# hila-chefer/Transformer-Explainability

Hardware: NVIDIA H100
Metric: explanations_per_sec (higher is better)
Workload: dtype f32

## Files before the change

include/te_b200.h:

```cpp
#ifndef TE_B200_H
#define TE_B200_H

#ifdef __cplusplus
extern "C" {
#endif

#if defined(__GNUC__)
#define TE_API __attribute__((visibility("default")))
#else
#define TE_API
#endif

#define TE_OK 0
#define TE_ERR_ARG (-1)
#define TE_ERR_WORKSPACE (-2)
#define TE_ERR_CUDA (-3)
#define TE_ERR_UNSUPPORTED (-4)

#define TE_FLAG_ZPLUS_TENSOR_CORES 1u
#define TE_FLAG_ROLLOUT_FUSED 2u
#define TE_FLAG_KEEP_ALL_CAMS 4u
#define TE_FLAG_LINEAR_TENSOR_CORES 16u
#define TE_FLAG_ATTN_TENSOR_CORES 32u
#define TE_FLAG_ZPLUS_BF16 64u
// ... 74 lines not shown
#define TE_BERT_ARCH_ROBERTA 1
#define TE_BERT_ARCH_DISTILBERT 2

TE_API int te_bert_num_weights(const te_bert_config* cfg);
TE_API const char* te_bert_weight_name(const te_bert_config* cfg, int i);
TE_API long long te_bert_weight_numel(const te_bert_config* cfg, int i);
TE_API long long te_bert_weight_offset(const te_bert_config* cfg, int i);
TE_API long long te_bert_weight_total(const te_bert_config* cfg);
TE_API long long te_bert_derived_total(const te_bert_config* cfg);
TE_API int te_bert_prepare_derived(const te_bert_config* cfg, const float* weights, float* derived, void* stream);
TE_API long long te_bert_workspace_bytes(const te_bert_config* cfg, int batch, int seq);

TE_API int te_bert_forward(const te_bert_config* cfg, const float* weights, const float* derived,
                    const long long* input_ids, const long long* attention_mask, const long long* token_type_ids,
                    int batch, int seq, unsigned flags, float* logits, void* workspace, long long workspace_bytes,
                    void* stream);
TE_API int te_bert_attribute(const te_bert_config* cfg, const float* weights, const float* derived, int batch, int seq,
                             int* index, int start_layer, float alpha, unsigned flags, float* maps, void* workspace,
                             long long workspace_bytes, void* stream);
TE_API int te_bert_explain(const te_bert_config* cfg, const float* weights, const float* derived,
                    const long long* input_ids, const long long* attention_mask, const long long* token_type_ids,
                    int batch, int seq, int* index, int start_layer, unsigned flags, float* maps, float* logits,
                    void* workspace, long long workspace_bytes, void* stream);
TE_API int te_bert_tensor(const te_bert_config* cfg, int batch, int seq, void* workspace, const char* name, int layer,
                   float** ptr, long long dims[4], long long strides[4]);

TE_API int te_linear_relprop(const float* x, const float* w, const float* bias, const float* y, const float* r, float* out,
                             float* scratch, int rows, int in_features, int out_features, float alpha, unsigned flags,
                             void* stream);
TE_API int te_add_relprop(const float* x1, const float* x2, const float* r, float* r1, float* r2, void* scratch,
                   int batch, long long per_sample, void* stream);
TE_API int te_clone_relprop(const float* x, const float* r1, const float* r2, const float* r3, float* out, long long n,
                     void* stream);
TE_API int te_matmul_av_relprop(const float* p, const float* v, const float* r, float* rp, float* rv, float* scratch,
                         int bh, int n, int d, void* stream);
TE_API int te_matmul_qk_relprop(const float* q, const float* k, const float* r, float* rq, float* rk, float* scratch,
                         int bh, int n, int d, void* stream);
TE_API int te_index_select_relprop(const float* x, const float* r, float* out, int batch, int n, int d, void* stream);
TE_API long long te_patch_embed_relprop_workspace_bytes(int batch, int in_chans, int img_size, int patch_size, int dim);
TE_API int te_patch_embed_relprop(const float* images, const float* weight, const float* r, int batch, int in_chans,
                           int img_size, int patch_size, int dim, float* r_pixels, float* r_sum, void* workspace,
                           long long workspace_bytes, void* stream);

TE_API int te_relevance_heatmap(const float* maps, int batch, int grid, int scale, float* out, void* stream);
TE_API int te_render_overlay(const float* images, const float* heat, int batch, int h, int w, int otsu, unsigned char* out,
                             int* thresholds, void* stream);
TE_API int te_head_reduce(const float* a, const float* g, const float* head_w, int batch, int heads, int n, int ld, int mode,
                   float* out, void* stream);
TE_API int te_head_region_mean(const float* g, int batch, int heads, int n, int ld, int r0, int r1, int c0, int c1, float* out,
                        void* stream);

TE_API long long te_rollout_workspace_bytes(int layers, int batch, int n);
TE_API int te_attribution_rollout(const float* grad, const float* cam, int layers, int batch, int heads, int n, int ld,
                           int start_layer, int normalize, unsigned flags, float* joint, float* row0,
                           void* workspace, long long workspace_bytes, void* stream);
TE_API int te_compute_rollout_attention(const float* mats, int layers, int batch, int n, int start_layer, int normalize,
                                 float* joint, void* workspace, long long workspace_bytes, void* stream);

TE_API int te_f16_block_split(const float* x, int rows, int cols, void* hi, void* lo, float* scale_inv, void* stream);

TE_API int te_linear_forward(const float* x, const float* w, const float* bias, const float* e0, float* y, float* y2,
                             float* scratch, int rows, int in_features, int out_features, int epi, unsigned flags,
                             void* stream);
TE_API int te_linear_backward(const float* dy, const float* w, const float* e0, float* dx, float* scratch, int rows,
                              int in_features, int out_features, int epi, unsigned flags, void* stream);
TE_API int te_layernorm_split(const float* x, const float* w, const float* b, float* y, float* mean, float* rstd, void* hi,
// ... 71 lines not shown
```

transformer_explainability_b200/_lib.py:

```python
import ctypes
import os

HERE = os.path.dirname(os.path.abspath(__file__))
LIB_PATH = os.path.join(HERE, "lib", "libte_b200.so")

c_int, c_ll, c_uint, c_void_p, c_char_p, c_float = (ctypes.c_int, ctypes.c_longlong, ctypes.c_uint, ctypes.c_void_p,
                                                    ctypes.c_char_p, ctypes.c_float)


class TeVitConfig(ctypes.Structure):
    _fields_ = [("img_size", c_int), ("patch_size", c_int), ("in_chans", c_int), ("num_classes", c_int),
                ("dim", c_int), ("depth", c_int), ("heads", c_int), ("mlp_dim", c_int), ("distilled", c_int),
                ("eps_block", c_float), ("eps_final", c_float)]


class TeBertConfig(ctypes.Structure):
    _fields_ = [("vocab_size", c_int), ("max_position", c_int), ("type_vocab", c_int), ("hidden", c_int),
                ("layers", c_int), ("heads", c_int), ("intermediate", c_int), ("num_labels", c_int),
                ("layer_norm_eps", c_float), ("arch", c_int), ("pad_token_id", c_int)]


BERT_ARCH_BERT = 0
BERT_ARCH_ROBERTA = 1
BERT_ARCH_DISTILBERT = 2
# ... 28 lines not shown
    "te_version": (c_int, []),
    "te_kernel_launch_count": (c_ll, []),
    "te_vit_num_weights": (c_int, [_CFG]),
    "te_vit_weight_name": (c_char_p, [_CFG, c_int]),
    "te_vit_weight_numel": (c_ll, [_CFG, c_int]),
    "te_vit_weight_offset": (c_ll, [_CFG, c_int]),
    "te_vit_weight_total": (c_ll, [_CFG]),
    "te_vit_workspace_bytes": (c_ll, [_CFG, c_int]),
    "te_vit_forward": (c_int, [_CFG, _P, _P, _P, c_int, c_uint, _P, _P, c_ll, _P]),
    "te_vit_derived_total": (c_ll, [_CFG]),
    "te_vit_prepare_derived": (c_int, [_CFG, _P, _P, _P]),
    "te_vit_attribute": (c_int, [_CFG, _P, _P, c_int, _P, c_int, c_float, c_uint, _P, _P, c_ll, _P]),
    "te_vit_explain": (c_int, [_CFG, _P, _P, _P, c_int, _P, c_int, c_uint, _P, _P, _P, c_ll, _P]),
    "te_vit_tensor": (c_int, [_CFG, c_int, _P, c_char_p, c_int, ctypes.POINTER(_P), ctypes.POINTER(c_ll),
                              ctypes.POINTER(c_ll)]),
    "te_set_option": (c_int, [c_char_p, c_int]),
    "te_vit_relprop_pixels": (c_int, [_CFG, _P, _P, c_int, c_uint, _P, _P, _P, c_ll, _P]),
    "te_bert_num_weights": (c_int, [_BCFG]),
    "te_bert_weight_name": (c_char_p, [_BCFG, c_int]),
    "te_bert_weight_numel": (c_ll, [_BCFG, c_int]),
    "te_bert_weight_offset": (c_ll, [_BCFG, c_int]),
    "te_bert_weight_total": (c_ll, [_BCFG]),
    "te_bert_derived_total": (c_ll, [_BCFG]),
    "te_bert_prepare_derived": (c_int, [_BCFG, _P, _P, _P]),
    "te_bert_workspace_bytes": (c_ll, [_BCFG, c_int, c_int]),
    "te_bert_forward": (c_int, [_BCFG, _P, _P, _P, _P, _P, c_int, c_int, c_uint, _P, _P, c_ll, _P]),
    "te_bert_attribute": (c_int, [_BCFG, _P, _P, c_int, c_int, _P, c_int, c_float, c_uint, _P, _P, c_ll, _P]),
    "te_bert_explain": (c_int, [_BCFG, _P, _P, _P, _P, _P, c_int, c_int, _P, c_int, c_uint, _P, _P, _P, c_ll, _P]),
    "te_bert_tensor": (c_int, [_BCFG, c_int, c_int, _P, c_char_p, c_int, ctypes.POINTER(_P), ctypes.POINTER(c_ll),
                               ctypes.POINTER(c_ll)]),
    "te_linear_relprop": (c_int, [_P, _P, _P, _P, _P, _P, _P, c_int, c_int, c_int, c_float, c_uint, _P]),
    "te_add_relprop": (c_int, [_P, _P, _P, _P, _P, _P, c_int, c_ll, _P]),
    "te_clone_relprop": (c_int, [_P, _P, _P, _P, _P, c_ll, _P]),
    "te_matmul_av_relprop": (c_int, [_P, _P, _P, _P, _P, _P, c_int, c_int, c_int, _P]),
    "te_matmul_qk_relprop": (c_int, [_P, _P, _P, _P, _P, _P, c_int, c_int, c_int, _P]),
    "te_index_select_relprop": (c_int, [_P, _P, _P, c_int, c_int, c_int, _P]),
    "te_patch_embed_relprop_workspace_bytes": (c_ll, [c_int, c_int, c_int, c_int, c_int]),
    "te_patch_embed_relprop": (c_int, [_P, _P, _P, c_int, c_int, c_int, c_int, c_int, _P, _P, _P, c_ll, _P]),
    "te_relevance_heatmap": (c_int, [_P, c_int, c_int, c_int, _P, _P]),
    "te_render_overlay": (c_int, [_P, _P, c_int, c_int, c_int, c_int, _P, _P, _P]),
    "te_head_reduce": (c_int, [_P, _P, _P, c_int, c_int, c_int, c_int, c_int, _P, _P]),
    "te_head_region_mean": (c_int, [_P, c_int, c_int, c_int, c_int, c_int, c_int, c_int, c_int, _P, _P]),
    "te_rollout_workspace_bytes": (c_ll, [c_int, c_int, c_int]),
    "te_attribution_rollout": (c_int, [_P, _P, c_int, c_int, c_int, c_int, c_int, c_int, c_int, c_uint, _P, _P, _P,
                                       c_ll, _P]),
    "te_compute_rollout_attention": (c_int, [_P, c_int, c_int, c_int, c_int, c_int, _P, _P, c_ll, _P]),
    "te_f16_block_split": (c_int, [_P, c_int, c_int, _P, _P, _P, _P]),
    "te_linear_forward": (c_int, [_P, _P, _P, _P, _P, _P, _P, c_int, c_int, c_int, c_int, c_uint, _P]),
    "te_linear_backward": (c_int, [_P, _P, _P, _P, _P, c_int, c_int, c_int, c_int, c_uint, _P]),
    "te_layernorm_split": (c_int, [_P, _P, _P, _P, _P, _P, _P, _P, _P, c_int, c_int, c_float, _P]),
    "te_tc_zplus_s": (c_int, [_P, _P, _P, _P, _P, _P, _P, _P, _P, c_int, c_int, c_int, c_uint, _P]),
    "te_tc_attention_nn": (c_int, [_P, c_ll, _P, c_ll, c_int, c_int, c_int, c_int, _P, c_int, _P, c_float, c_int, c_int, _P]),
    "te_tc_attention_nk": (c_int, [_P, c_int, c_int, _P, c_ll, c_int, c_int, c_int, _P, c_int, _P, c_float, c_int, c_int, _P]),
    "te_perturb_workspace_bytes": (c_ll, [c_int, c_ll]),
    "te_perturb_images": (c_int, [_P, _P, c_int, c_int, c_ll, ctypes.POINTER(c_int), c_int, c_int, ctypes.POINTER(c_float),
                                  ctypes.POINTER(c_float), _P, _P, c_ll, _P]),
    "te_logit_stats": (c_int, [_P, _P, c_int, c_int, _P, _P, _P, _P, _P]),
    "te_sort_workspace_bytes": (c_ll, [c_ll, c_int]),
    "te_sort_keys_u32": (c_int, [_P, _P, c_ll, c_int, _P, c_ll, _P]),
    "te_seg_workspace_bytes": (c_ll, [c_int, c_int, c_int]),
    "te_seg_metrics": (c_int, [_P, _P, c_int, c_int, c_int, c_float, _P, _P, _P, _P, _P, _P, _P, _P, c_ll, _P]),
    "te_pr_curve_workspace_bytes": (c_ll, [c_ll]),
    "te_pr_curve": (c_int, [_P, c_ll, _P, _P, _P, _P, _P, c_ll, _P]),
    "te_eraser_workspace_bytes": (c_ll, [c_int, c_ll, c_ll]),
    "te_eraser_rationales": (c_int, [_P, c_int, c_int, _P, _P, _P, _P, _P, c_int, _P, c_int, _P, _P, _P, _P, c_ll, _P]),
    "te_eraser_reduce_workspace_bytes": (c_ll, [c_int, c_ll, c_int]),
# ... 66 lines not shown
```

transformer_explainability_b200/csrc/te_api.cu:

```cuda
#include <stdlib.h>
#include <string.h>
#include <atomic>
#include <string>

#include "../../include/te_b200.h"
#include "te_engine_util.h"
#include "te_kernels.h"
#include "te_rollout.h"
#include "te_zplus.h"
#include "te_gemm_tc.h"

static thread_local std::string g_last_error;
void te_set_last_error(const char* msg) { g_last_error = msg ? msg : ""; }

static std::atomic<long long> g_launches{0};
void te_count_launch() { g_launches.fetch_add(1, std::memory_order_relaxed); }
extern "C" long long te_kernel_launch_count(void) { return g_launches.load(); }

extern "C" const char* te_last_error(void) { return g_last_error.c_str(); }
extern "C" int te_version(void) { return 101; }

#define ST(s) reinterpret_cast<cudaStream_t>(s)
#define REQ(c, msg) do { if (!(c)) { te_set_last_error(msg); return TE_ERR_ARG; } } while (0)

// ... 132 lines not shown

extern "C" int te_linear_relprop(const float* x, const float* w, const float* bias, const float* y, const float* r, float* out,
                                 float* scratch, int rows, int in_features, int out_features, float alpha, unsigned flags,
                                 void* stream) {
    REQ(x && w && r && out && scratch && rows > 0 && in_features > 0 && out_features > 0, "te_linear_relprop: bad argument");
    REQ(isfinite(alpha), "te_linear_relprop: alpha must be finite");
    const bool lrp = (flags & TE_FLAG_RULES_LRP) != 0;
    const float* derived = nullptr;
    float* xabs = nullptr;
    if ((flags & (lrp ? TE_FLAG_RULES_LRP_TC : TE_FLAG_ZPLUS_TENSOR_CORES)) &&
        te_tc_zplus_supported(rows, in_features, out_features, in_features)) {
        const TcScratch c = tc_scratch(scratch, (long long)rows * out_features, in_features, out_features, 0);
        TE_TRY(te_tc_prepare_weights(w, c.derived, in_features, out_features, ST(stream)));
        derived = c.derived;
        if (y) xabs = c.op;
    }
    return te_linear_rule_relprop(lrp, x, in_features, w, derived, r, out_features, out, scratch, rows, in_features, out_features,
                                  ST(stream), y, out_features, bias, y ? te_zplus_from_flags(flags) : ZplusVariant{}, 0, xabs,
                                  alpha);
}

extern "C" int te_add_relprop(const float* x1, const float* x2, const float* r, float* r1, float* r2, void* scratch,
                              int batch, long long per_sample, void* stream) {
    REQ(x1 && x2 && r && r1 && r2 && batch > 0 && per_sample > 0, "te_add_relprop: bad argument");
    return te_launch_add_relprop(x1, x2, r, r1, r2, reinterpret_cast<double*>(scratch), batch, per_sample, ST(stream));
}

extern "C" int te_clone_relprop(const float* x, const float* r1, const float* r2, const float* r3, float* out,
                                long long n, void* stream) {
    REQ(x && r1 && r2 && out && n > 0, "te_clone_relprop: bad argument");
    return te_launch_clone_relprop(x, r1, r2, r3, out, n, ST(stream));
}

extern "C" int te_index_select_relprop(const float* x, const float* r, float* out, int batch, int n, int d,
                                       void* stream) {
    REQ(x && r && out && batch > 0 && n > 0 && d > 0, "te_index_select_relprop: bad argument");
    return te_launch_index_select_relprop(x, r, nullptr, out, batch, n, d, ST(stream));
}

extern "C" int te_matmul_av_relprop(const float* p_, const float* v, const float* r, float* rp, float* rv,
                                    float* scratch, int bh, int n, int d, void* stream) {
    REQ(p_ && v && r && rp && rv && scratch && bh > 0 && n > 0 && d > 0 && d % 4 == 0, "te_matmul_av_relprop: bad argument");
    cudaStream_t st = ST(stream);
    const long long nn = (long long)n * n, nd = (long long)n * d;
    TeGemm g = g0(bh);
    g.A = p_; g.lda = n; g.sA1 = nn; g.B = v; g.ldb = d; g.sB1 = nd; g.C = scratch; g.ldc = d; g.sC1 = nd;
    g.M = n; g.N = d; g.K = n;
    TE_TRY(te_gemm_launch(g, TE_L_K, TE_L_MN, TE_XF_NONE, TE_EPI_STORE, st));
    TE_TRY(te_launch_sd(r, scratch, scratch, (long long)bh * nd, st));
    g = g0(bh);
    g.A = scratch; g.lda = d; g.sA1 = nd; g.B = v; g.ldb = d; g.sB1 = nd; g.C = rp; g.ldc = n; g.sC1 = nn;
    g.E0 = p_; g.lde0 = n; g.sE1 = nn; g.M = n; g.N = n; g.K = d;
    TE_TRY(te_gemm_launch(g, TE_L_K, TE_L_K, TE_XF_NONE, TE_EPI_MUL, st));
    g = g0(bh);
    g.A = p_; g.lda = n; g.sA1 = nn; g.B = scratch; g.ldb = d; g.sB1 = nd; g.C = rv; g.ldc = d; g.sC1 = nd;
    g.E0 = v; g.lde0 = d; g.sE1 = nd; g.M = n; g.N = d; g.K = n;
    TE_TRY(te_gemm_launch(g, TE_L_MN, TE_L_MN, TE_XF_NONE, TE_EPI_MUL, st));
    return TE_OK;
}

extern "C" int te_matmul_qk_relprop(const float* q, const float* k, const float* r, float* rq, float* rk,
                                    float* scratch, int bh, int n, int d, void* stream) {
    REQ(q && k && r && rq && rk && scratch && bh > 0 && n > 0 && d > 0, "te_matmul_qk_relprop: bad argument");
    cudaStream_t st = ST(stream);
    const long long nn = (long long)n * n, nd = (long long)n * d;
    TeGemm g = g0(bh);
// ... 124 lines not shown
```

transformer_explainability_b200/csrc/te_bert.cu:

```cuda
#include <string.h>

#include <algorithm>

#include "../../include/te_b200.h"
#include "te_engine_util.h"
#include "te_gemm_tc.h"
#include "te_kernels.h"
#include "te_rollout.h"
#include "te_zplus.h"

using namespace te_util;

namespace {

constexpr int kMaxDepth = 64;

struct Dims {
    int B, N, NP, D, H, dh, F, C, L, V, P, T, arch, pad;
    long long M;
    float eps;
};

static bool make_dims(const te_bert_config* c, int B, int S, Dims& d) {
    if (!c || c->layers <= 0 || c->layers > kMaxDepth || c->heads <= 0 || c->hidden % c->heads != 0 || c->hidden % 8 != 0 ||
// ... 326 lines not shown
        TE_TRY(linear_bwd_tc(tw.qkv, dqkv, lw.qkvw, dxn, nullptr, d.M, d.D, 3 * d.D, TE_EPI_STORE, st, sel.btf, &sel.bfs));
        TE_TRY(te_launch_add2(dxn, dsx, dxa, MD, st));
    }

    if (flags & TE_FLAG_GRADIENTS_ONLY) return TE_OK;
    const long long layer_stride = d.L > 1 ? (long long)(ws.layer[1].G - ws.layer[0].G) : 0;
    if (grad_rollout) {
        TE_TRY(te_rollout_layers(ws.layer[0].G, ws.layer[0].P, layer_stride, d.L, d.B, d.H, d.N, d.NP, d.NP, start_layer,
                                 0, flags, ws.mats, ws.joint[0], ws.joint[1], nullptr, maps, 0,
                                 0, st));
        if (cudaMemset2DAsync(maps, sizeof(float) * d.N, 0, sizeof(float), d.B, st) != cudaSuccess) {
            te_set_last_error("te_bert_attribute: clearing element 0 of the maps failed");
            return TE_ERR_CUDA;
        }
        return TE_OK;
    }

    float* R = ws.tD[0]; float* R1 = ws.tD[1]; float* R2 = ws.tD[2]; float* R3 = ws.tD[3];
    float* RF = ws.tF[0]; float* SF = ws.tF[1]; float* S = ws.t3D[0]; float* Rqkv = ws.t3D[1];
    double* addp = sel.lrp ? nullptr : ws.addpart;
    TE_TRY(te_linear_rule_relprop(sel.lrp, ws.pooled, d.D, w.clsw, nullptr, ws.seed, d.C, ws.rpool, ws.shead, d.B, d.D, d.C, st,
                                  nullptr, 0, nullptr, sel.zv, 0, nullptr, alpha));
    TE_TRY(te_linear_rule_relprop(sel.lrp, ws.h_last, (long long)d.N * d.D, w.poolw, nullptr, ws.rpool, d.D, ws.rfirst, ws.shead,
                                  d.B, d.D, d.D, st, nullptr, 0, nullptr, sel.zv, 0, nullptr, alpha));
    TE_TRY(te_launch_index_select_relprop(ws.h_last, ws.rfirst, nullptr, R, d.B, d.N, d.D, st));

    for (int l = d.L - 1; l >= sel.low; --l) {
        LayerAct& a = ws.layer[l];
        const LayerW& lw = w.layer[l];
        const DerivedW dw = bind_derived(d, sel.dbase, l);
        const bool top = (l == d.L - 1) && te_engine_cls_rows();
        const long long zr = top ? d.B : d.M;
        const long long sD = top ? (long long)d.N * d.D : d.D, sF = top ? (long long)d.N * d.F : d.F;
        TE_TRY(te_launch_add_relprop(a.d2, a.ao, R, R1, R2, addp, d.B, (long long)d.N * d.D, st));
        TE_TRY(te_linear_rule_relprop(sel.lrp, a.g, sF, lw.w2, dw.w2, R1, sD, RF, S, zr, d.F, d.D, st, a.d2, sD, lw.b2, sel.zv, sF,
                                      SF, alpha));
        TE_TRY(te_linear_rule_relprop(sel.lrp, a.ao, sD, lw.w1, dw.w1, RF, sF, R1, SF, zr, d.D, d.F, st, a.hpre, sF, lw.b1, sel.zv,
                                      sD, S, alpha));
        TE_TRY(te_launch_clone_relprop(a.ao, R1, R2, nullptr, R, MD, st));
        TE_TRY(te_launch_add_relprop(a.d1, a.h, R, R1, R2, addp, d.B, (long long)d.N * d.D, st));
        if (top) TE_TRY(te_launch_fill(R3, 0.f, MD, st));
        TE_TRY(te_linear_rule_relprop(sel.lrp, a.ctx, sD, lw.ow, dw.o, R1, sD, R3, S, zr, d.D, d.D, st, a.d1, sD, lw.ob, sel.zv, sD,
                                      S + MD, alpha));
        const bool last = (l == sel.low && !(flags & TE_FLAG_RELPROP_TO_INPUT));
        TE_TRY(attn_relprop_pv(sel, d.B, d.H, d.N, d.NP, d.dh, a.qkv, a.P, R3, a.ctx, S, a.cam, Rqkv, last, st));
        if (last) break;
        TE_TRY(attn_nn(sel.atc, d.B, d.H, d.N, d.NP, d.dh, a.qkv, 3 * d.D, a.qkv + d.D, 3 * d.D, ws.tA[0], nullptr, scale,
                       TE_EPI_STORE, st));
        TE_TRY(te_launch_add_relprop_keymask(ws.tA[0], ws.maskadd, a.cam, ws.tA[1], addp, d.B, d.H, d.N, d.NP, st));
        TE_TRY(attn_relprop_qk(sel, d.B, d.H, d.N, d.NP, d.dh, a.qkv, ws.tA[1], ws.tA[0], Rqkv, st));
        TE_TRY(te_linear_rule_relprop(sel.lrp, a.h, d.D, lw.qkvw, dw.q, Rqkv, 3 * d.D, R, S, d.M, d.D, d.D, st, a.qkv, 3 * d.D,
                                      lw.qkvb, sel.zv, 0, S + MD, alpha));
        TE_TRY(te_linear_rule_relprop(sel.lrp, a.h, d.D, lw.qkvw + DD, dw.k, Rqkv + d.D, 3 * d.D, R1, S, d.M, d.D, d.D, st,
                                      a.qkv + d.D, 3 * d.D, lw.qkvb + d.D, sel.zv, 0, S + MD, alpha));
        TE_TRY(te_linear_rule_relprop(sel.lrp, a.h, d.D, lw.qkvw + 2 * DD, dw.v, Rqkv + 2 * d.D, 3 * d.D, R3, S, d.M, d.D, d.D, st,
                                      a.qkv + 2 * d.D, 3 * d.D, lw.qkvb + 2 * d.D, sel.zv, 0, S + MD, alpha));
        TE_TRY(te_launch_clone_relprop(a.h, R, R1, R3, SF, MD, st));
        TE_TRY(te_launch_clone_relprop(a.h, SF, R2, nullptr, R, MD, st));
    }

    TE_TRY(te_rollout_layers(ws.layer[0].G, ws.layer[0].cam, layer_stride, d.L, d.B, d.H, d.N, d.NP, d.NP, start_layer,
                             1, flags, ws.mats, ws.joint[0], ws.joint[1], nullptr, maps, 0,
                             1, st));
    return TE_OK;
}

extern "C" int te_bert_explain(const te_bert_config* cfg, const float* weights, const float* derived,
                               const long long* input_ids, const long long* attention_mask,
                               const long long* token_type_ids, int batch, int seq, int* index, int start_layer,
                               unsigned flags, float* maps, float* logits, void* workspace, long long workspace_bytes,
                               void* stream) {
    TE_TRY(te_bert_forward(cfg, weights, derived, input_ids, attention_mask, token_type_ids, batch, seq, flags, logits,
                           workspace, workspace_bytes, stream));
    return te_bert_attribute(cfg, weights, derived, batch, seq, index, start_layer, 1.f, flags, maps, workspace, workspace_bytes,
                             stream);
}

extern "C" int te_bert_tensor(const te_bert_config* cfg, int batch, int seq, void* workspace, const char* name, int layer,
                              float** ptr, long long dims[4], long long strides[4]) {
    Dims d; Workspace ws;
    if (!workspace || !name || !ptr) return TE_ERR_ARG;
    if (batch <= 0 || !make_dims(cfg, batch, seq, d)) return TE_ERR_ARG;
    carve(d, reinterpret_cast<char*>(workspace), ws);
    const std::string n(name);
    const View set{ptr, dims, strides};
    if (n == "logits") return set(ws.logits, d.B, d.C, 1, 1, d.C, 1, 1, 1);
    if (n == "relevance_in") return set(ws.tD[0], d.B, d.N, d.D, 1, (long long)d.N * d.D, d.D, 1, 1);
    if (n.rfind("tmp_d", 0) == 0 && n.size() == 6 && n[5] >= '0' && n[5] <= '3')
        return set(ws.tD[n[5] - '0'], d.B, d.N, d.D, 1, (long long)d.N * d.D, d.D, 1, 1);
    if (n.rfind("tmp_f", 0) == 0 && n.size() == 6 && n[5] >= '0' && n[5] <= '1')
        return set(ws.tF[n[5] - '0'], d.B, d.N, d.F, 1, (long long)d.N * d.F, d.F, 1, 1);
// ... 24 lines not shown
```

transformer_explainability_b200/csrc/te_kernels.h:

```cpp
#pragma once
#include "te_common.cuh"
#include "te_gemm.cuh"

int te_launch_im2col(const float* img, float* patches, int B, int C, int H, int W, int P, cudaStream_t st);
int te_launch_assemble_tokens(const float* patch_out, const float* cls, const float* dist, const float* pos,
                              float* x, int B, int N, int D, int n_prefix, cudaStream_t st);
int te_launch_layernorm(const float* x, const float* w, const float* b, float* y, float* mean, float* rstd,
                        long long rows, int D, float eps, cudaStream_t st);
int te_launch_layernorm_split(const float* x, const float* w, const float* b, float* y, float* mean, float* rstd,
                              long long rows, int D, float eps, float* split, float* scale, cudaStream_t st);
int te_launch_layernorm_bwd(const float* dy, const float* x, const float* w, const float* mean, const float* rstd,
                            const float* dres, float* dx, long long rows, int D, cudaStream_t st);
int te_launch_layernorm_bwd_strided(const float* dy, long long dy_stride, const float* x, long long x_stride,
                                    const float* w, float eps, float* dx, long long dx_stride, int rows, int D,
                                    cudaStream_t st);
int te_launch_softmax(float* s, long long rows, int N, int ld, cudaStream_t st);
int te_launch_softmax_bwd(const float* p, const float* dp, float* ds, long long rows, int N, int ld, float scale,
                          cudaStream_t st);
int te_launch_argmax(const float* logits, int* index, int B, int C, int only_negative, cudaStream_t st);
int te_launch_average2(const float* a, const float* b, float* out, long long n, cudaStream_t st);
int te_launch_onehot(const int* index, float* seed, int B, int C, float value, cudaStream_t st);
int te_launch_sd(const float* a, const float* b, float* out, long long n, cudaStream_t st);
int te_launch_clone_relprop(const float* x, const float* r1, const float* r2, const float* r3, float* out,
                            long long n, cudaStream_t st);
#define TE_ADD_SPLIT 16
int te_launch_add_relprop(const float* x1, const float* x2, const float* r, float* r1, float* r2, double* partial,
                          int B, long long per_sample, cudaStream_t st);
int te_launch_add_relprop_strided(const float* x1, const float* x2, long long x2_sample_stride, const float* r, float* r1,
                                  float* r2, double* partial, int B, long long per_sample, cudaStream_t st);
long long te_patch_relprop_scratch_floats(int B, int C, int img, int P, int D);
int te_patch_relprop_run(const float* images, const float* weight, const float* r, long long r_sample_stride, int B,
                         int C, int img, int P, int D, float* scratch, float* r_pixels, float* r_sum, cudaStream_t st);
int te_launch_index_select_relprop(const float* x, const float* r_tok0, const float* r_tok1, float* out, int B,
                                   int N, int D, cudaStream_t st);
int te_launch_aggregate(const float* G, const float* cam, float* M, int B, int H, int N, int ld_in, int ld_out,
                        int add_eye, int normalize, cudaStream_t st, float* diag = nullptr);
int te_launch_aggregate_layers(const float* G0, const float* cam0, long long in_layer_stride, float* M0, long long m_layer_stride,
                               int B, int H, int N, int ld_in, int ld_out, int first_layer, int num_layers, int normalize,
                               cudaStream_t st, float* diag0 = nullptr);
int te_launch_relevance_heatmap(const float* maps, float* out, int B, int g, int scale, cudaStream_t st);
int te_launch_head_reduce(const float* a, const float* g, const float* hw, float* out, int B, int H, int N, int ld,
                          int mode, cudaStream_t st);
int te_launch_head_region_mean(const float* g, float* out, int BH, int N, int ld, int r0, int r1, int c0, int c1,
                               cudaStream_t st);
int te_launch_prep_mats(const float* in, float* out, long long rows, int N, int ld_in, int ld_out, int normalize,
                        cudaStream_t st);
int te_launch_extract_row(const float* joint, float* out, int B, int N, int ld, int first, int bert_fix,
                          cudaStream_t st);
int te_launch_fill(float* p, float v, long long n, cudaStream_t st);
int te_launch_softmax_masked(float* s, long long rows, int N, int ld, const float* keymask, long long rows_per_batch,
                             cudaStream_t st);
int te_launch_bert_embed(const long long* ids, const long long* token_type_ids, const float* word, const float* pos,
                         const float* type, float* out, int B, int S, int D, int vocab, int type_vocab, cudaStream_t st);
int te_launch_hf_embed(const long long* ids, const long long* token_type_ids, const float* word, const float* pos,
                       const float* type, float* out, int B, int S, int D, int vocab, int max_position, int type_vocab,
                       int pad, cudaStream_t st);
int te_launch_bert_mask(const long long* mask, float* out, long long n, cudaStream_t st);
int te_launch_tanh(const float* x, float* y, long long n, cudaStream_t st);
int te_launch_tanh_bwd(const float* dy, const float* y, float* dx, long long n, cudaStream_t st);
int te_launch_relu(const float* x, float* y, long long n, cudaStream_t st);
int te_launch_relu_bwd(const float* dy, const float* y, float* dx, long long n, cudaStream_t st);
int te_launch_add2(const float* a, const float* b, float* out, long long n, cudaStream_t st);
// ... 3 lines not shown
```

transformer_explainability_b200/csrc/te_vit.cu:

```cuda
#include <string.h>

#include <algorithm>

#include "../../include/te_b200.h"
#include "te_engine_util.h"
#include "te_kernels.h"
#include "te_rollout.h"
#include "te_zplus.h"
#include "te_gemm_tc.h"

namespace {

constexpr int kMaxDepth = 64;

struct Dims {
    int B, N, NP, D, H, dh, F, C, L, P, img, Cin, npatch, prefix, KP;
    long long M;
};

static bool make_dims(const te_vit_config* c, int B, Dims& d) {
    if (!c || c->depth <= 0 || c->depth > kMaxDepth || c->heads <= 0 || c->dim % c->heads != 0 || c->dim % 4 != 0 ||
        c->mlp_dim % 4 != 0 || c->patch_size % 4 != 0 || c->img_size % c->patch_size != 0 || c->num_classes <= 0) {
        te_set_last_error("te_vit: invalid config");
        return false;
// ... 282 lines not shown
        if (cfg->distilled) {
            TE_TRY(linear_bwd(ws.seed, w.headdw, ws.dpool, nullptr, d.B, d.D, d.C, TE_EPI_STORE, st));
            TE_TRY(te_launch_layernorm_bwd_strided(ws.dpool, d.D, ws.x_last + d.D, (long long)d.N * d.D, w.normw,
                                                   cfg->eps_final, dxa + d.D, (long long)d.N * d.D, d.B, d.D, st));
        }
    }
    for (int l = d.L - 1; l >= start_layer; --l) {
        LayerAct& a = ws.layer[l];
        const BlockW& bw = w.blk[l];
        const DerivedW lw = bind_derived(d, sel.lbase, l);
        TE_TRY(te_util::linear_bwd_tc(lw.fc2, dxa, bw.fc2w, dF, a.h, d.M, d.F, d.D, TE_EPI_GELU_BWD, st, sel.btf, &sel.bfs));
        TE_TRY(te_util::linear_bwd_tc(lw.fc1, dF, bw.fc1w, dxn, nullptr, d.M, d.D, d.F, TE_EPI_STORE, st, sel.btf, &sel.bfs));
        TE_TRY(te_launch_layernorm_bwd(dxn, a.x_mid, bw.n2w, a.mean2, a.rstd2, dxa, dxb, d.M, d.D, st));
        TE_TRY(te_util::linear_bwd_tc(lw.proj, dxb, bw.projw, dctx, nullptr, d.M, d.D, d.D, TE_EPI_STORE, st, sel.btf, &sel.bfs));
        const bool last = (l == start_layer);
        TE_TRY(te_util::attn_block_bwd(sel, d.B, d.H, d.N, d.NP, d.dh, a.qkv, a.P, dctx, a.G, dS, dqkv, scale, last, st));
        if (last) break;
        TE_TRY(te_util::linear_bwd_tc(lw.qkv, dqkv, bw.qkvw, dxn, nullptr, d.M, d.D, 3 * d.D, TE_EPI_STORE, st, sel.btf, &sel.bfs));
        TE_TRY(te_launch_layernorm_bwd(dxn, a.x_in, bw.n1w, a.mean1, a.rstd1, dxb, dxa, d.M, d.D, st));
    }

    if (flags & TE_FLAG_GRADIENTS_ONLY) return TE_OK;
    const long long layer_stride = d.L > 1 ? (long long)(ws.layer[1].G - ws.layer[0].G) : 0;
    if (grad_rollout)
        return te_rollout_layers(ws.layer[0].G, ws.layer[0].P, layer_stride, d.L, d.B, d.H, d.N, d.NP, d.NP, start_layer,
                                 0, flags, ws.mats, ws.joint[0], ws.joint[1], nullptr, maps, d.prefix,
                                 0, st);

    float* R = ws.tD[0]; float* R1 = ws.tD[1]; float* R2 = ws.tD[2]; float* R3 = ws.tD[3];
    float* RF = ws.tF[0]; float* SF = ws.tF[1]; float* S = ws.t3D[0]; float* Rqkv = ws.t3D[1]; float* S1 = ws.tA;
    auto addrule = [&](const float* x1, const float* x2, const float* r, float* r1, float* r2) -> int {
        return te_launch_add_relprop(x1, x2, r, r1, r2, sel.lrp ? nullptr : ws.addpart, d.B, (long long)d.N * d.D, st);
    };
    TE_TRY(te_linear_rule_relprop(sel.lrp, ws.xf, (long long)d.N * d.D, w.headw, nullptr, ws.seed, d.C, ws.rhead0, ws.shead, d.B,
                                  d.D, d.C, st, nullptr, 0, nullptr, sel.zv, 0, nullptr, alpha));
    if (cfg->distilled)
        TE_TRY(te_linear_rule_relprop(sel.lrp, ws.xf + d.D, (long long)d.N * d.D, w.headdw, nullptr, ws.seed, d.C, ws.rhead1,
                                      ws.shead, d.B, d.D, d.C, st, nullptr, 0, nullptr, sel.zv, 0, nullptr, alpha));
    TE_TRY(te_launch_index_select_relprop(ws.xf, ws.rhead0, cfg->distilled ? ws.rhead1 : nullptr, R, d.B, d.N, d.D, st));

    for (int l = d.L - 1; l >= sel.low; --l) {
        LayerAct& a = ws.layer[l];
        const BlockW& bw = w.blk[l];
        const DerivedW dw = bind_derived(d, sel.dbase, l);
        const bool top = (l == d.L - 1) && !cfg->distilled && !sel.lrp && te_engine_cls_rows();
        const long long zr = top ? d.B : d.M;
        const long long sD = top ? (long long)d.N * d.D : d.D, sF = top ? (long long)d.N * d.F : d.F;
        TE_TRY(addrule(a.x_mid, a.mlp_out, R, R1, R2));
        TE_TRY(te_linear_rule_relprop(sel.lrp, a.g, sF, bw.fc2w, dw.fc2, R2, sD, RF, S, zr, d.F, d.D, st, a.mlp_out, sD, bw.fc2b,
                                      sel.zv, sF, SF, alpha));
        TE_TRY(te_linear_rule_relprop(sel.lrp, a.xn2, sD, bw.fc1w, dw.fc1, RF, sF, R2, SF, zr, d.D, d.F, st, a.h, sF, bw.fc1b,
                                      sel.zv, sD, S, alpha));
        TE_TRY(te_launch_clone_relprop(a.x_mid, R1, R2, nullptr, R, MD, st));
        TE_TRY(addrule(a.x_in, a.attn_out, R, R1, R2));
        if (top) TE_TRY(te_launch_fill(R3, 0.f, MD, st));
        TE_TRY(te_linear_rule_relprop(sel.lrp, a.ctx, sD, bw.projw, dw.proj, R2, sD, R3, S, zr, d.D, d.D, st, a.attn_out, sD,
                                      bw.projb, sel.zv, sD, S + MD, alpha));
        const bool last = (l == sel.low && !(flags & TE_FLAG_RELPROP_TO_INPUT));
        TE_TRY(te_util::attn_relprop_pv(sel, d.B, d.H, d.N, d.NP, d.dh, a.qkv, a.P, R3, a.ctx, S, a.cam, Rqkv, last, st));
        if (last) break;
        TE_TRY(te_util::attn_relprop_qk(sel, d.B, d.H, d.N, d.NP, d.dh, a.qkv, a.cam, S1, Rqkv, st));
        TE_TRY(te_linear_rule_relprop(sel.lrp, a.xn1, d.D, bw.qkvw, dw.qkv, Rqkv, 3 * d.D, R2, S, d.M, d.D, 3 * d.D, st, a.qkv,
                                      3 * d.D, bw.qkvb, sel.zv, 0, RF, alpha));
        TE_TRY(te_launch_clone_relprop(a.x_in, R1, R2, nullptr, R, MD, st));
    }

    TE_TRY(te_rollout_layers(ws.layer[0].G, ws.layer[0].cam, layer_stride, d.L, d.B, d.H, d.N, d.NP, d.NP,
                             start_layer, 0, flags, ws.mats, ws.joint[0], ws.joint[1], nullptr, maps,
                             d.prefix, 0, st));
    return TE_OK;
}

extern "C" int te_vit_relprop_pixels(const te_vit_config* cfg, const float* weights, const float* images, int batch,
                                     unsigned flags, float* pixel_maps, float* pixel_relevance, void* workspace,
                                     long long workspace_bytes, void* stream) {
    Dims d; Workspace ws;
    TE_TRY(check_ws(cfg, batch, workspace, workspace_bytes, d, ws));
    if (!weights || !images || (!pixel_maps && !pixel_relevance)) { te_set_last_error("te_vit_relprop_pixels: null pointer"); return TE_ERR_ARG; }
    cudaStream_t st = reinterpret_cast<cudaStream_t>(stream);
    Weights w;
    bind_weights(cfg, weights, w);
    float* R = ws.tD[0];
    float* tokens = ws.tD[1];
    float* Rtok = ws.tD[2];
    float* patches = ws.tF[0];
    float* patch_out = ws.tD[3];
    TE_TRY(te_launch_im2col(images, patches, d.B, d.Cin, d.img, d.img, d.P, st));
    TE_TRY(linear_fwd(patches, d.KP, w.patchw, w.patchb, patch_out, nullptr, nullptr, (long long)d.B * d.npatch, d.KP,
                      d.D, TE_EPI_BIAS, st));
    TE_TRY(te_launch_assemble_tokens(patch_out, w.cls, w.dist, nullptr, tokens, d.B, d.N, d.D, d.prefix, st));
    TE_TRY(te_launch_add_relprop_strided(tokens, w.pos, 0, R, Rtok, nullptr, (flags & TE_FLAG_RULES_LRP) ? nullptr : ws.addpart,
                                         d.B, (long long)d.N * d.D, st));
    return te_patch_relprop_run(images, w.patchw, Rtok + (long long)d.prefix * d.D, (long long)d.N * d.D, d.B, d.Cin, d.img,
                                d.P, d.D, ws.pix, pixel_relevance, pixel_maps, st);
}

extern "C" int te_vit_explain(const te_vit_config* cfg, const float* weights, const float* derived, const float* images,
// ... 47 lines not shown
```

transformer_explainability_b200/ops.py:

```python
import torch

from . import _lib
from ._lib import check, ptr


import functools


def _stream():
    return _lib.ctypes.c_void_p(torch.cuda.current_stream().cuda_stream)


def _on_device(fn):
    @functools.wraps(fn)
    def wrapped(*args, **kwargs):
        dev = None
        for a in list(args) + list(kwargs.values()):
            if isinstance(a, (list, tuple)) and a and torch.is_tensor(a[0]):
                a = a[0]
            if torch.is_tensor(a) and a.is_cuda:
                dev = a.device
                break
        if dev is None:
            raise ValueError("te_b200 ops need CUDA tensors (no CPU fallback)")
# ... 228 lines not shown
        raise ValueError("variant: 'ours', 'lrp' or 'lrp_tc'")
    check(_lib.load().te_linear_relprop(ptr(x), ptr(w), ptr(bias) if y is not None else None, ptr(y), ptr(r), ptr(out),
                                        ptr(scratch), rows, x.shape[-1], w.shape[0], float(alpha), flags, _stream()),
          "te_linear_relprop")
    return out


@_on_device
def add_relprop(x1, x2, r, variant="ours"):
    _req(x1, x2, r)
    _same_shape("add_relprop", x1, x2, r)
    if (x1.numel() // max(x1.shape[0], 1)) % 4 != 0:
        raise ValueError("add_relprop: elements per sample must be a multiple of 4")
    b = x1.shape[0]
    r1, r2 = torch.empty_like(x1), torch.empty_like(x1)
    scratch = None if variant == "lrp" else torch.empty(b * 48, device=x1.device, dtype=torch.float64)
    check(_lib.load().te_add_relprop(ptr(x1), ptr(x2), ptr(r), ptr(r1), ptr(r2), ptr(scratch), b, x1.numel() // b,
                                     _stream()), "te_add_relprop")
    return r1, r2


@_on_device
def clone_relprop(x, rs):
    rs = list(rs)
    _req(x, *rs)
    if len(rs) not in (2, 3):
        raise ValueError("clone_relprop: 2 or 3 branches")
    _same_shape("clone_relprop", x, *rs)
    out = torch.empty_like(x)
    r3 = rs[2] if len(rs) > 2 else None
    check(_lib.load().te_clone_relprop(ptr(x), ptr(rs[0]), ptr(rs[1]), ptr(r3), ptr(out), x.numel(), _stream()),
          "te_clone_relprop")
    return out


@_on_device
def index_select_relprop(x, r):
    if x.dim() != 3 or r.numel() != x.shape[0] * x.shape[2]:
        raise ValueError("index_select_relprop: x [B,N,D], r [B,1,D] expected")
    r = r.reshape(x.shape[0], x.shape[2]).contiguous()
    _req(x, r)
    out = torch.empty_like(x)
    check(_lib.load().te_index_select_relprop(ptr(x), ptr(r), ptr(out), x.shape[0], x.shape[1], x.shape[2], _stream()),
          "te_index_select_relprop")
    return out


@_on_device
def matmul_av_relprop(p, v, r):
    _req(p, v, r)
    if v.dim() != 4 or p.shape != v.shape[:2] + (v.shape[2], v.shape[2]):
        raise ValueError("matmul_av_relprop: p [B,H,N,N], v [B,H,N,d], r [B,H,N,d] expected")
    _same_shape("matmul_av_relprop", v, r)
    b, h, n, d = v.shape
    rp, rv = torch.empty_like(p), torch.empty_like(v)
    scratch = torch.empty(b * h * n * d, device=p.device, dtype=torch.float32)
    check(_lib.load().te_matmul_av_relprop(ptr(p), ptr(v), ptr(r), ptr(rp), ptr(rv), ptr(scratch), b * h, n, d,
                                           _stream()), "te_matmul_av_relprop")
    return rp, rv


@_on_device
def matmul_qk_relprop(q, k, r):
    _req(q, k, r)
    if q.dim() != 4 or r.shape != q.shape[:2] + (q.shape[2], q.shape[2]):
        raise ValueError("matmul_qk_relprop: q, k [B,H,N,d], r [B,H,N,N] expected")
# ... 417 lines not shown
```

Before: 924.5.

## Fuse residual clone and add relevance propagation into one cluster kernel

Adds a kernel that merges each clone_relprop with the following add_relprop, in both the ViT and BERT backward relevance loops. Per-sample normalization is done with a thread-block cluster reduction over distributed shared memory, and the intermediates are kept in shared memory so they are not written to and re-read from global memory. This removes one kernel launch and several full-tensor round trips per residual junction. The cost is large dynamic shared memory with one CTA per SM, and a fallback to the two separate kernels when the per-sample data does not fit.

```diff
diff --git a/include/te_b200.h b/include/te_b200.h
--- a/include/te_b200.h
+++ b/include/te_b200.h
@@ -130,6 +130,9 @@
                    int batch, long long per_sample, void* stream);
 TE_API int te_clone_relprop(const float* x, const float* r1, const float* r2, const float* r3, float* out, long long n,
                      void* stream);
+TE_API int te_clone_add_relprop(const float* x, const float* c1, const float* c2, const float* x1, const float* x2,
+                                float* r1, float* r2, void* scratch, int batch, long long per_sample, int x_is_sum,
+                                void* stream);
 TE_API int te_matmul_av_relprop(const float* p, const float* v, const float* r, float* rp, float* rv, float* scratch,
                          int bh, int n, int d, void* stream);
 TE_API int te_matmul_qk_relprop(const float* q, const float* k, const float* r, float* rq, float* rk, float* scratch,
diff --git a/transformer_explainability_b200/_lib.py b/transformer_explainability_b200/_lib.py
--- a/transformer_explainability_b200/_lib.py
+++ b/transformer_explainability_b200/_lib.py
@@ -84,6 +84,7 @@
     "te_linear_relprop": (c_int, [_P, _P, _P, _P, _P, _P, _P, c_int, c_int, c_int, c_float, c_uint, _P]),
     "te_add_relprop": (c_int, [_P, _P, _P, _P, _P, _P, c_int, c_ll, _P]),
     "te_clone_relprop": (c_int, [_P, _P, _P, _P, _P, c_ll, _P]),
+    "te_clone_add_relprop": (c_int, [_P, _P, _P, _P, _P, _P, _P, _P, c_int, c_ll, c_int, _P]),
     "te_matmul_av_relprop": (c_int, [_P, _P, _P, _P, _P, _P, c_int, c_int, c_int, _P]),
     "te_matmul_qk_relprop": (c_int, [_P, _P, _P, _P, _P, _P, c_int, c_int, c_int, _P]),
     "te_index_select_relprop": (c_int, [_P, _P, _P, c_int, c_int, c_int, _P]),
diff --git a/transformer_explainability_b200/csrc/te_api.cu b/transformer_explainability_b200/csrc/te_api.cu
--- a/transformer_explainability_b200/csrc/te_api.cu
+++ b/transformer_explainability_b200/csrc/te_api.cu
@@ -188,6 +188,16 @@
     return te_launch_clone_relprop(x, r1, r2, r3, out, n, ST(stream));
 }
 
+extern "C" int te_clone_add_relprop(const float* x, const float* c1, const float* c2, const float* x1, const float* x2,
+                                    float* r1, float* r2, void* scratch, int batch, long long per_sample, int x_is_sum,
+                                    void* stream) {
+    REQ(x && c1 && c2 && x1 && x2 && r1 && r2 && batch > 0 && per_sample > 0, "te_clone_add_relprop: bad argument");
+    double* partial = reinterpret_cast<double*>(scratch);
+    float* r_tmp = scratch ? reinterpret_cast<float*>(partial + (long long)batch * TE_ADD_SPLIT * 3) : nullptr;
+    return te_launch_clone_add_relprop(x, c1, c2, x1, x2, r1, r2, partial, r_tmp, batch, per_sample, x_is_sum != 0,
+                                       ST(stream));
+}
+
 extern "C" int te_index_select_relprop(const float* x, const float* r, float* out, int batch, int n, int d,
                                        void* stream) {
     REQ(x && r && out && batch > 0 && n > 0 && d > 0, "te_index_select_relprop: bad argument");
diff --git a/transformer_explainability_b200/csrc/te_bert.cu b/transformer_explainability_b200/csrc/te_bert.cu
--- a/transformer_explainability_b200/csrc/te_bert.cu
+++ b/transformer_explainability_b200/csrc/te_bert.cu
@@ -382,13 +382,15 @@
         const bool top = (l == d.L - 1) && te_engine_cls_rows();
         const long long zr = top ? d.B : d.M;
         const long long sD = top ? (long long)d.N * d.D : d.D, sF = top ? (long long)d.N * d.F : d.F;
-        TE_TRY(te_launch_add_relprop(a.d2, a.ao, R, R1, R2, addp, d.B, (long long)d.N * d.D, st));
+        if (l == d.L - 1) TE_TRY(te_launch_add_relprop(a.d2, a.ao, R, R1, R2, addp, d.B, (long long)d.N * d.D, st));
+        else TE_TRY(te_launch_clone_add_relprop(ws.layer[l + 1].h, SF, R2, a.d2, a.ao, R1, R2, addp, R, d.B,
+                                                (long long)d.N * d.D, false, st));
         TE_TRY(te_linear_rule_relprop(sel.lrp, a.g, sF, lw.w2, dw.w2, R1, sD, RF, S, zr, d.F, d.D, st, a.d2, sD, lw.b2, sel.zv, sF,
                                       SF, alpha));
         TE_TRY(te_linear_rule_relprop(sel.lrp, a.ao, sD, lw.w1, dw.w1, RF, sF, R1, SF, zr, d.D, d.F, st, a.hpre, sF, lw.b1, sel.zv,
                                       sD, S, alpha));
-        TE_TRY(te_launch_clone_relprop(a.ao, R1, R2, nullptr, R, MD, st));
-        TE_TRY(te_launch_add_relprop(a.d1, a.h, R, R1, R2, addp, d.B, (long long)d.N * d.D, st));
+        TE_TRY(te_launch_clone_add_relprop(a.ao, R1, R2, a.d1, a.h, R1, R2, addp, R, d.B, (long long)d.N * d.D, false,
+                                           st));
         if (top) TE_TRY(te_launch_fill(R3, 0.f, MD, st));
         TE_TRY(te_linear_rule_relprop(sel.lrp, a.ctx, sD, lw.ow, dw.o, R1, sD, R3, S, zr, d.D, d.D, st, a.d1, sD, lw.ob, sel.zv, sD,
                                       S + MD, alpha));
@@ -406,7 +408,8 @@
         TE_TRY(te_linear_rule_relprop(sel.lrp, a.h, d.D, lw.qkvw + 2 * DD, dw.v, Rqkv + 2 * d.D, 3 * d.D, R3, S, d.M, d.D, d.D, st,
                                       a.qkv + 2 * d.D, 3 * d.D, lw.qkvb + 2 * d.D, sel.zv, 0, S + MD, alpha));
         TE_TRY(te_launch_clone_relprop(a.h, R, R1, R3, SF, MD, st));
-        TE_TRY(te_launch_clone_relprop(a.h, SF, R2, nullptr, R, MD, st));
+        if (l == sel.low)
+            TE_TRY(te_launch_clone_relprop(a.h, SF, R2, nullptr, R, MD, st));
     }
 
     TE_TRY(te_rollout_layers(ws.layer[0].G, ws.layer[0].cam, layer_stride, d.L, d.B, d.H, d.N, d.NP, d.NP, start_layer,
diff --git a/transformer_explainability_b200/csrc/te_kernels.h b/transformer_explainability_b200/csrc/te_kernels.h
--- a/transformer_explainability_b200/csrc/te_kernels.h
+++ b/transformer_explainability_b200/csrc/te_kernels.h
@@ -28,6 +28,9 @@
                           int B, long long per_sample, cudaStream_t st);
 int te_launch_add_relprop_strided(const float* x1, const float* x2, long long x2_sample_stride, const float* r, float* r1,
                                   float* r2, double* partial, int B, long long per_sample, cudaStream_t st);
+int te_launch_clone_add_relprop(const float* x, const float* c1, const float* c2, const float* x1, const float* x2,
+                                float* r1, float* r2, double* partial, float* r_tmp, int B, long long per_sample,
+                                bool x_is_sum, cudaStream_t st);
 long long te_patch_relprop_scratch_floats(int B, int C, int img, int P, int D);
 int te_patch_relprop_run(const float* images, const float* weight, const float* r, long long r_sample_stride, int B,
                          int C, int img, int P, int D, float* scratch, float* r_pixels, float* r_sum, cudaStream_t st);
diff --git a/transformer_explainability_b200/csrc/te_residual.cu b/transformer_explainability_b200/csrc/te_residual.cu
--- /dev/null
+++ b/transformer_explainability_b200/csrc/te_residual.cu
@@ -0,0 +1,185 @@
+#include <cooperative_groups.h>
+
+#include "te_kernels.h"
+
+namespace cg = cooperative_groups;
+
+namespace {
+
+constexpr int kSplitThreads = 256;
+constexpr int kSplitsPerCta = 2;
+constexpr int kCluster = TE_ADD_SPLIT / kSplitsPerCta;
+constexpr int kThreads = kSplitThreads * kSplitsPerCta;
+constexpr int kFlatThreads = 256;
+
+__device__ __forceinline__ void clone_add_elem(float4 xv, float4 a, float4 b, float4 u, float4 v, float4& r, float4& pa,
+                                               float4& pb) {
+    const float4 c = make_float4(te_sd(a.x, xv.x) + te_sd(b.x, xv.x), te_sd(a.y, xv.y) + te_sd(b.y, xv.y),
+                                 te_sd(a.z, xv.z) + te_sd(b.z, xv.z), te_sd(a.w, xv.w) + te_sd(b.w, xv.w));
+    r = make_float4(xv.x * c.x, xv.y * c.y, xv.z * c.z, xv.w * c.w);
+    const float s0 = te_sd(r.x, u.x + v.x), s1 = te_sd(r.y, u.y + v.y);
+    const float s2 = te_sd(r.z, u.z + v.z), s3 = te_sd(r.w, u.w + v.w);
+    pa = make_float4(u.x * s0, u.y * s1, u.z * s2, u.w * s3);
+    pb = make_float4(v.x * s0, v.y * s1, v.z * s2, v.w * s3);
+}
+
+template <bool SUM>
+__device__ __forceinline__ float4 clone_input(const float4* x, long long t, float4 u, float4 v) {
+    if (SUM) return make_float4(u.x + v.x, u.y + v.y, u.z + v.z, u.w + v.w);
+    return x[t];
+}
+
+template <bool SUM>
+__global__ void clone_add_lrp_kernel(const float* __restrict__ x, const float* c1, const float* c2,
+                                     const float* __restrict__ x1, const float* __restrict__ x2, float* r1, float* r2,
+                                     long long n4) {
+    for (long long t = blockIdx.x * (long long)blockDim.x + threadIdx.x; t < n4;
+         t += (long long)gridDim.x * blockDim.x) {
+        float4 r, pa, pb;
+        const float4 u = reinterpret_cast<const float4*>(x1)[t], v = reinterpret_cast<const float4*>(x2)[t];
+        clone_add_elem(clone_input<SUM>(reinterpret_cast<const float4*>(x), t, u, v), reinterpret_cast<const float4*>(c1)[t],
+                       reinterpret_cast<const float4*>(c2)[t], u, v, r, pa, pb);
+        reinterpret_cast<float4*>(r1)[t] = pa;
+        reinterpret_cast<float4*>(r2)[t] = pb;
+    }
+}
+
+template <bool SUM>
+__global__ void __cluster_dims__(kCluster, 1, 1) __launch_bounds__(kThreads, 1)
+clone_add_kernel(const float* __restrict__ x, const float* c1, const float* c2, const float* __restrict__ x1,
+                 const float* __restrict__ x2, float* r1, float* r2, long long per4) {
+    extern __shared__ float4 kept[];
+    __shared__ double part[kSplitsPerCta][3];
+    __shared__ double red[kSplitsPerCta][3][kSplitThreads / 32];
+    __shared__ float fa_s, fb_s;
+    cg::cluster_group cluster = cg::this_cluster();
+    const int half = threadIdx.x / kSplitThreads, tid = threadIdx.x % kSplitThreads;
+    const int b = blockIdx.x / kCluster;
+    const int sp = (int)cluster.block_rank() * kSplitsPerCta + half;
+    const long long chunk = (per4 + TE_ADD_SPLIT - 1) / TE_ADD_SPLIT;
+    const long long lo = sp * chunk, hi = min(per4, lo + chunk);
+    const long long base = b * per4;
+    float4* ka = kept + (long long)half * 2 * chunk;
+    float4* kb = ka + chunk;
+
+    const float4 *px = reinterpret_cast<const float4*>(x) + base, *pc1 = reinterpret_cast<const float4*>(c1) + base;
+    const float4 *pc2 = reinterpret_cast<const float4*>(c2) + base, *pu = reinterpret_cast<const float4*>(x1) + base;
+    const float4* pv = reinterpret_cast<const float4*>(x2) + base;
+    double sa = 0.0, sb = 0.0, sr = 0.0;
+    long long t = lo + tid;
+    float4 nx = make_float4(0.f, 0.f, 0.f, 0.f), na, nb, nu, nv;
+    if (t < hi) { if (!SUM) nx = px[t]; na = pc1[t]; nb = pc2[t]; nu = pu[t]; nv = pv[t]; }
+    for (; t < hi; t += kSplitThreads) {
+        const float4 a = na, c = nb, u = nu, v = nv;
+        const float4 xv = SUM ? clone_input<true>(px, t, u, v) : nx;
+        const long long tn = t + kSplitThreads;
+        if (tn < hi) { if (!SUM) nx = px[tn]; na = pc1[tn]; nb = pc2[tn]; nu = pu[tn]; nv = pv[tn]; }
+        float4 rr, pa, pb;
+        clone_add_elem(xv, a, c, u, v, rr, pa, pb);
+        sa += ((double)pa.x + (double)pa.y) + ((double)pa.z + (double)pa.w);
+        sb += ((double)pb.x + (double)pb.y) + ((double)pb.z + (double)pb.w);
+        sr += ((double)rr.x + (double)rr.y) + ((double)rr.z + (double)rr.w);
+        ka[t - lo] = pa;
+        kb[t - lo] = pb;
+    }
+    sa = te_warp_sum(sa); sb = te_warp_sum(sb); sr = te_warp_sum(sr);
+    const int lane = tid & 31, wid = tid >> 5;
+    if (lane == 0) { red[half][0][wid] = sa; red[half][1][wid] = sb; red[half][2][wid] = sr; }
+    __syncthreads();
+    if (tid == 0) {
+        double ta = 0, tb = 0, tr = 0;
+        for (int i = 0; i < kSplitThreads / 32; ++i) { ta += red[half][0][i]; tb += red[half][1][i]; tr += red[half][2][i]; }
+        part[half][0] = ta; part[half][1] = tb; part[half][2] = tr;
+    }
+    cluster.sync();
+
+    if (threadIdx.x == 0) {
+        double A = 0, Bs = 0, rho = 0;
+        for (int i = 0; i < TE_ADD_SPLIT; ++i) {
+            const double* q = &cluster.map_shared_rank(&part[0][0], i / kSplitsPerCta)[(i % kSplitsPerCta) * 3];
+            A += q[0]; Bs += q[1]; rho += q[2];
+        }
+        const double den = fabs(A) + fabs(Bs);
+        const double a_fact = te_sd(fabs(A), den) * rho;
+        const double b_fact = te_sd(fabs(Bs), den) * rho;
+        fa_s = (float)te_sd(a_fact, A);
+        fb_s = (float)te_sd(b_fact, Bs);
+    }
+    cluster.sync();
+
+    const float fa = fa_s, fb = fb_s;
+    for (t = lo + tid; t < hi; t += kSplitThreads) {
+        const float4 pa = ka[t - lo], pb = kb[t - lo];
+        reinterpret_cast<float4*>(r1)[base + t] = make_float4(pa.x * fa, pa.y * fa, pa.z * fa, pa.w * fa);
+        reinterpret_cast<float4*>(r2)[base + t] = make_float4(pb.x * fb, pb.y * fb, pb.z * fb, pb.w * fb);
+    }
+}
+
+long long fused_smem_limit() {
+    static long long limit[64];
+    static unsigned long long done = 0;
+    int dev = 0;
+    if (cudaGetDevice(&dev) != cudaSuccess) return 0;
+    if (done & (1ull << (dev & 63))) return limit[dev & 63];
+    int optin = 0;
+    long long lim = 0;
+    cudaFuncAttributes fa;
+    if (cudaDeviceGetAttribute(&optin, cudaDevAttrMaxSharedMemoryPerBlockOptin, dev) == cudaSuccess &&
+        cudaFuncGetAttributes(&fa, clone_add_kernel<false>) == cudaSuccess) {
+        const int dyn = optin - (int)fa.sharedSizeBytes;
+        if (cudaFuncSetAttribute(clone_add_kernel<false>, cudaFuncAttributeMaxDynamicSharedMemorySize, dyn) == cudaSuccess &&
+            cudaFuncSetAttribute(clone_add_kernel<true>, cudaFuncAttributeMaxDynamicSharedMemorySize, dyn) == cudaSuccess) {
+            cudaLaunchConfig_t cfg;
+            memset(&cfg, 0, sizeof(cfg));
+            cfg.gridDim = dim3(kCluster);
+            cfg.blockDim = dim3(kThreads);
+            cfg.dynamicSmemBytes = dyn;
+            cudaLaunchAttribute attr[1];
+            attr[0].id = cudaLaunchAttributeClusterDimension;
+            attr[0].val.clusterDim.x = kCluster;
+            attr[0].val.clusterDim.y = 1;
+            attr[0].val.clusterDim.z = 1;
+            cfg.attrs = attr;
+            cfg.numAttrs = 1;
+            int clusters = 0;
+            if (cudaOccupancyMaxActiveClusters(&clusters, clone_add_kernel<false>, &cfg) == cudaSuccess && clusters > 0) lim = dyn;
+        }
+    }
+    cudaGetLastError();
+    limit[dev & 63] = lim;
+    done |= 1ull << (dev & 63);
+    return lim;
+}
+
+long long kept_bytes(long long per_sample) {
+    const long long chunk = (per_sample / 4 + TE_ADD_SPLIT - 1) / TE_ADD_SPLIT;
+    return (long long)kSplitsPerCta * 2 * chunk * (long long)sizeof(float4);
+}
+
+}
+
+int te_launch_clone_add_relprop(const float* x, const float* c1, const float* c2, const float* x1, const float* x2,
+                                float* r1, float* r2, double* partial, float* r_tmp, int B, long long per_sample,
+                                bool x_is_sum, cudaStream_t st) {
+    if (per_sample % 4 != 0) { te_set_last_error("clone_add_relprop: per-sample size % 4 != 0"); return TE_ERR_ARG; }
+    const long long per4 = per_sample / 4;
+    if (partial == nullptr) {
+        const long long n4 = (long long)B * per4;
+        long long g = (n4 + kFlatThreads - 1) / kFlatThreads;
+        g = g < 1 ? 1 : (g > 132LL * 16 ? 132LL * 16 : g);
+        if (x_is_sum) clone_add_lrp_kernel<true><<<(int)g, kFlatThreads, 0, st>>>(x, c1, c2, x1, x2, r1, r2, n4);
+        else clone_add_lrp_kernel<false><<<(int)g, kFlatThreads, 0, st>>>(x, c1, c2, x1, x2, r1, r2, n4);
+        TE_CUDA_CHECK_LAUNCH();
+        return TE_OK;
+    }
+    if (kept_bytes(per_sample) > fused_smem_limit()) {
+        TE_TRY(te_launch_clone_relprop(x, c1, c2, nullptr, r_tmp, (long long)B * per_sample, st));
+        return te_launch_add_relprop(x1, x2, r_tmp, r1, r2, partial, B, per_sample, st);
+    }
+    if ((long long)B * kCluster > 0x7fffffffLL) { te_set_last_error("clone_add_relprop: batch too large"); return TE_ERR_ARG; }
+    const long long smem = kept_bytes(per_sample);
+    if (x_is_sum) clone_add_kernel<true><<<B * kCluster, kThreads, smem, st>>>(x, c1, c2, x1, x2, r1, r2, per4);
+    else clone_add_kernel<false><<<B * kCluster, kThreads, smem, st>>>(x, c1, c2, x1, x2, r1, r2, per4);
+    TE_CUDA_CHECK_LAUNCH();
+    return TE_OK;
+}
diff --git a/transformer_explainability_b200/csrc/te_vit.cu b/transformer_explainability_b200/csrc/te_vit.cu
--- a/transformer_explainability_b200/csrc/te_vit.cu
+++ b/transformer_explainability_b200/csrc/te_vit.cu
@@ -338,6 +338,10 @@
     auto addrule = [&](const float* x1, const float* x2, const float* r, float* r1, float* r2) -> int {
         return te_launch_add_relprop(x1, x2, r, r1, r2, sel.lrp ? nullptr : ws.addpart, d.B, (long long)d.N * d.D, st);
     };
+    auto clone_add = [&](const float* x, const float* x1, const float* x2) -> int {
+        return te_launch_clone_add_relprop(x, R1, R2, x1, x2, R1, R2, sel.lrp ? nullptr : ws.addpart, R, d.B,
+                                           (long long)d.N * d.D, true, st);
+    };
     TE_TRY(te_linear_rule_relprop(sel.lrp, ws.xf, (long long)d.N * d.D, w.headw, nullptr, ws.seed, d.C, ws.rhead0, ws.shead, d.B,
                                   d.D, d.C, st, nullptr, 0, nullptr, sel.zv, 0, nullptr, alpha));
     if (cfg->distilled)
@@ -352,13 +356,13 @@
         const bool top = (l == d.L - 1) && !cfg->distilled && !sel.lrp && te_engine_cls_rows();
         const long long zr = top ? d.B : d.M;
         const long long sD = top ? (long long)d.N * d.D : d.D, sF = top ? (long long)d.N * d.F : d.F;
-        TE_TRY(addrule(a.x_mid, a.mlp_out, R, R1, R2));
+        if (l == d.L - 1) TE_TRY(addrule(a.x_mid, a.mlp_out, R, R1, R2));
+        else TE_TRY(clone_add(ws.layer[l + 1].x_in, a.x_mid, a.mlp_out));
         TE_TRY(te_linear_rule_relprop(sel.lrp, a.g, sF, bw.fc2w, dw.fc2, R2, sD, RF, S, zr, d.F, d.D, st, a.mlp_out, sD, bw.fc2b,
                                       sel.zv, sF, SF, alpha));
         TE_TRY(te_linear_rule_relprop(sel.lrp, a.xn2, sD, bw.fc1w, dw.fc1, RF, sF, R2, SF, zr, d.D, d.F, st, a.h, sF, bw.fc1b,
                                       sel.zv, sD, S, alpha));
-        TE_TRY(te_launch_clone_relprop(a.x_mid, R1, R2, nullptr, R, MD, st));
-        TE_TRY(addrule(a.x_in, a.attn_out, R, R1, R2));
+        TE_TRY(clone_add(a.x_mid, a.x_in, a.attn_out));
         if (top) TE_TRY(te_launch_fill(R3, 0.f, MD, st));
         TE_TRY(te_linear_rule_relprop(sel.lrp, a.ctx, sD, bw.projw, dw.proj, R2, sD, R3, S, zr, d.D, d.D, st, a.attn_out, sD,
                                       bw.projb, sel.zv, sD, S + MD, alpha));
@@ -368,7 +372,8 @@
         TE_TRY(te_util::attn_relprop_qk(sel, d.B, d.H, d.N, d.NP, d.dh, a.qkv, a.cam, S1, Rqkv, st));
         TE_TRY(te_linear_rule_relprop(sel.lrp, a.xn1, d.D, bw.qkvw, dw.qkv, Rqkv, 3 * d.D, R2, S, d.M, d.D, 3 * d.D, st, a.qkv,
                                       3 * d.D, bw.qkvb, sel.zv, 0, RF, alpha));
-        TE_TRY(te_launch_clone_relprop(a.x_in, R1, R2, nullptr, R, MD, st));
+        if (l == sel.low)
+            TE_TRY(te_launch_clone_relprop(a.x_in, R1, R2, nullptr, R, MD, st));
     }
 
     TE_TRY(te_rollout_layers(ws.layer[0].G, ws.layer[0].cam, layer_stride, d.L, d.B, d.H, d.N, d.NP, d.NP,
diff --git a/transformer_explainability_b200/ops.py b/transformer_explainability_b200/ops.py
--- a/transformer_explainability_b200/ops.py
+++ b/transformer_explainability_b200/ops.py
@@ -284,6 +284,26 @@
     check(_lib.load().te_clone_relprop(ptr(x), ptr(rs[0]), ptr(rs[1]), ptr(r3), ptr(out), x.numel(), _stream()),
           "te_clone_relprop")
     return out
+
+
+@_on_device
+def clone_add_relprop(x, rs, x1, x2, variant="ours", x_is_sum=False):
+    rs = list(rs)
+    _req(x, x1, x2, *rs)
+    if len(rs) != 2:
+        raise ValueError("clone_add_relprop: 2 clone branches")
+    _same_shape("clone_add_relprop", x, x1, x2, *rs)
+    if (x1.numel() // max(x1.shape[0], 1)) % 4 != 0:
+        raise ValueError("clone_add_relprop: elements per sample must be a multiple of 4")
+    b = x1.shape[0]
+    r1, r2 = torch.empty_like(x1), torch.empty_like(x1)
+    scratch = None
+    if variant != "lrp":
+        scratch = torch.empty(b * 48 + (x1.numel() + 1) // 2, device=x1.device, dtype=torch.float64)
+    check(_lib.load().te_clone_add_relprop(ptr(x), ptr(rs[0]), ptr(rs[1]), ptr(x1), ptr(x2), ptr(r1), ptr(r2),
+                                           ptr(scratch), b, x1.numel() // b, int(bool(x_is_sum)), _stream()),
+          "te_clone_add_relprop")
+    return r1, r2
 
 
 @_on_device
```

After: 941.9, median of 6. 1.02x the previous value.
